# khuzema-h/marl-gym-pybullet-drones

Hardware: NVIDIA B200
Metric: drone_substeps_per_sec (higher is better)
Workload: dtype f32

## Files before the change

### marl_gym_pybullet_drones_b200/build.py

```python
from __future__ import annotations

import os
import shutil
import subprocess
import sys

_HERE = os.path.dirname(os.path.abspath(__file__))
CSRC = os.path.join(_HERE, "csrc")
SOURCES = [os.path.join(CSRC, "bd_kernels.cu"), os.path.join(CSRC, "bd_tile_launch.cu"), os.path.join(CSRC, "bd_api.cu"), os.path.join(CSRC, "bd_actor.cu"),
           os.path.join(CSRC, "bd_norm.cu"), os.path.join(CSRC, "bd_ppo.cu"), os.path.join(CSRC, "bd_peer.cu")]
HEADERS = [os.path.join(CSRC, "bd_params.h"), os.path.join(CSRC, "bd_device.cuh"), os.path.join(CSRC, "bd_step_tile.cuh"),
           os.path.join(CSRC, "bd_umma.cuh"),
           os.path.join(os.path.dirname(_HERE), "include", "batch_drones.h")]
OUT = os.path.join(_HERE, "libbatchdrones.so")

NVCC_FLAGS = [
    "-gencode", "arch=compute_100a,code=sm_100a",
    "-O3", "-lineinfo", "-std=c++17",
    "-Xcompiler", "-fPIC", "-shared",
]


def find_nvcc() -> str:
    cand = shutil.which("nvcc") or "/usr/local/cuda/bin/nvcc"
    if not os.path.exists(cand):
        raise RuntimeError("nvcc not found; cannot build the CUDA extension")
    return cand


def up_to_date() -> bool:
    if not os.path.exists(OUT):
        return False
    t = os.path.getmtime(OUT)
    return all(os.path.getmtime(p) <= t for p in SOURCES + HEADERS)


def build(force: bool = False, verbose: bool = False) -> str:
    if not force and up_to_date():
        return OUT
    from concurrent.futures import ThreadPoolExecutor
    nvcc = find_nvcc()
    objdir = os.path.join(CSRC, "_obj")
    os.makedirs(objdir, exist_ok=True)
    compile_flags = [f for f in NVCC_FLAGS if f != "-shared"]

    def compile_one(src):
        obj = os.path.join(objdir, os.path.basename(src)[:-3] + ".o")
        cmd = [nvcc] + compile_flags + (["-Xptxas", "-v"] if verbose else []) + ["-c", "-o", obj, src]
        res = subprocess.run(cmd, capture_output=True, text=True)
        if res.returncode != 0:
            raise RuntimeError("nvcc failed on " + src + ":\n" + res.stdout + res.stderr)
        if verbose:
            print(res.stderr)
        return obj

    with ThreadPoolExecutor(max_workers=len(SOURCES)) as pool:
        objs = list(pool.map(compile_one, SOURCES))
    res = subprocess.run([nvcc] + NVCC_FLAGS + ["-o", OUT] + objs, capture_output=True, text=True)
    if res.returncode != 0:
        raise RuntimeError("nvcc link failed:\n" + res.stdout + res.stderr)
    return OUT


if __name__ == "__main__":
    print(build(force="--force" in sys.argv, verbose="-v" in sys.argv))
```

### marl_gym_pybullet_drones_b200/csrc/bd_step_tile.cuh

```cuda
#pragma once
#include "bd_device.cuh"

namespace bd {

template <int A>
struct TileIn {
  float4 s0, s1, s2, s3;
  float4 act;
  int stepc;
  float ep_ret;
};

template <int A, bool HINT = false>
__device__ __forceinline__ void load_state(const Params<float>& P, long long g, int env, bool active, TileIn<A>& in,
                                           const L2Hints& h = L2Hints{}) {
  if (active) {
    if constexpr (HINT) {
      in.s0 = ld_hint(P.s0 + g, h.state); in.s1 = ld_hint(P.s1 + g, h.state);
      in.s2 = ld_hint(P.s2 + g, h.state); in.s3 = ld_hint(P.s3 + g, h.state);
      in.stepc = ld_hint(P.stepc + env, h.state);
      in.ep_ret = P.ep_ret != nullptr ? ld_hint(P.ep_ret + env, h.state) : 0.f;
    } else {
      in.s0 = P.s0[g]; in.s1 = P.s1[g]; in.s2 = P.s2[g]; in.s3 = P.s3[g];
      in.stepc = P.stepc[env];
      in.ep_ret = P.ep_ret != nullptr ? P.ep_ret[env] : 0.f;
    }
  } else {
    in.s0 = in.s1 = in.s2 = in.s3 = make_float4(0.f, 0.f, 0.f, 0.f);
    in.s1.z = 1.0f;
    in.stepc = 0;
    in.ep_ret = 0.f;
  }
}
template <int A, bool HINT = false>
__device__ __forceinline__ void load_action(const Params<float>& P, long long g, bool active, TileIn<A>& in,
                                            const L2Hints& h = L2Hints{}) {
  if (active) {
    if constexpr (HINT) {
      if constexpr (A == 4) in.act = ld_hint(reinterpret_cast<const float4*>(P.actions) + g, h.once);
      else in.act = make_float4(ld_hint(reinterpret_cast<const float*>(P.actions) + g, h.once), 0.f, 0.f, 0.f);
    } else {
      if constexpr (A == 4) in.act = reinterpret_cast<const float4*>(P.actions)[g];
      else in.act = make_float4(reinterpret_cast<const float*>(P.actions)[g], 0.f, 0.f, 0.f);
    }
  } else {
    in.act = make_float4(0.f, 0.f, 0.f, 0.f);
  }
}

__device__ __forceinline__ float swarm_reward_shfl(const Params<float>& P, const Drone<float>& d, float roll, float pitch,
                                                   int lane, int M, int drone, int& flags) {
  const unsigned full = 0xffffffffu;
  const int base = lane & ~(M - 1);
  const bool tilt = fabsf(roll) > .4f || fabsf(pitch) > .4f;
  flags = 0;
  float contrib = 0.f;
  if (P.task == TASK_MEETUP) {
    const int src = base | (M - 1 - drone);
    const float ox = __shfl_sync(full, d.px, src), oy = __shfl_sync(full, d.py, src), oz = __shfl_sync(full, d.pz, src);
    if (drone < M / 2) {
      const float dx = d.px - ox, dy = d.py - oy, dz = d.pz - oz;
      const float dist = sqrtf(dx * dx + dy * dy + dz * dz);
      contrib = (-1.f * (dist * dist)) * 2.f;
      if (dist > 0.1f) flags |= 4;
    }
    if (fabsf(d.px) > 5.0f || fabsf(d.py) > 5.0f || d.pz > 3.0f || d.pz < 0.1f || tilt) flags |= 2;
  } else if (P.task == TASK_LEADERFOLLOWER) {
    const float z0 = __shfl_sync(full, d.pz, base);
    if (drone == 0) {
      const float ex = 0.f - d.px, ey = 0.f - d.py, ez = 0.5f - d.pz;
      const float n = sqrtf(ex * ex + ey * ey + ez * ez);
      contrib = -1.f * (n * n);
    } else {
      const float dz = z0 - d.pz;
      const float n = sqrtf(dz * dz);
      contrib = -(1.f / (float)M) * (n * n);
    }
    if (fabsf(d.px) > 2.0f || fabsf(d.py) > 2.0f || d.pz > 2.0f || tilt) flags |= 2;
  } else {
    const float eps = 1e-3f;
    const float ni = sqrtf(d.vx * d.vx + d.vy * d.vy + d.vz * d.vz);
    float ali = 0.f, sp = 0.f;
#pragma unroll 1
    for (int o = 1; o < M; ++o) {
      const int src = base | ((lane + o) & (M - 1));
      const float ox = __shfl_sync(full, d.px, src), oy = __shfl_sync(full, d.py, src), oz = __shfl_sync(full, d.pz, src);
      const float ux = __shfl_sync(full, d.vx, src), uy = __shfl_sync(full, d.vy, src), uz = __shfl_sync(full, d.vz, src);
      const float nj = __shfl_sync(full, ni, src);
      const float dot = d.vx * ux + d.vy * uy + d.vz * uz;
      ali += dot / (ni + eps) / (nj + eps);
      const float dx = ox - d.px, dy = oy - d.py, dz = oz - d.pz;
      const float dist = sqrtf(dx * dx + dy * dy + dz * dz);
      sp = (o == 1 || dist < sp) ? dist : sp;
    }
    if (fabsf(d.px) > 10.0f || fabsf(d.py) > 10.0f || d.pz > 10.0f || tilt) flags |= 2;
    float cx = d.vx, cy = d.vy, cz = d.vz, ssp = sp;
#pragma unroll 1
    for (int o = M >> 1; o > 0; o >>= 1) {
      ali += __shfl_xor_sync(full, ali, o);
      cx += __shfl_xor_sync(full, cx, o); cy += __shfl_xor_sync(full, cy, o); cz += __shfl_xor_sync(full, cz, o);
      ssp += __shfl_xor_sync(full, ssp, o);
    }
    cx /= (float)M; cy /= (float)M; cz /= (float)M;
    const float speed = sqrtf(cx * cx + cy * cy + cz * cz);
    if (M == 1) return speed;
    const float avg = ssp / (float)M;
    float var = (sp - avg) * (sp - avg);
#pragma unroll 1
    for (int o = M >> 1; o > 0; o >>= 1) var += __shfl_xor_sync(full, var, o);
    var /= (float)M;
    float pen = 0.f;
    if (!(1.0f < avg && avg < 3.0f)) {
      const float a = fabsf(avg - 1.0f), b = fabsf(avg - 3.0f);
      pen = a < b ? a : b;
    }
    return ((ali / (float)(M * (M - 1)) + speed) - pen) - var;
  }
#pragma unroll 1
  for (int o = M >> 1; o > 0; o >>= 1) contrib += __shfl_xor_sync(full, contrib, o);
  return contrib;
}

template <int TASK, int A, bool VEC, int AERO>
__global__ void __launch_bounds__(kBlock, 6)
step_kernel_tile(const __grid_constant__ Params<float> P) {
  extern __shared__ __align__(128) unsigned char smem_raw[];
  const int tid = threadIdx.x, lane = tid & 31;
  const int M = P.M, B = P.B, D = P.D, EW = P.EW;
  const bool pow2 = (M & (M - 1)) == 0;
  constexpr bool vec = VEC;
  float* tile_s = reinterpret_cast<float*>(smem_raw);
  const int env_w = pow2 ? (lane >> (31 - __clz(M))) : lane / M;
  const int group_base = env_w * M;
  const int drone = lane - group_base;
  const int tile = blockIdx.x + P.block0;
  const int env_l = (tid >> 5) * EW + env_w;
  const int env = tile * (4 * EW) + env_l;
  const bool active = env_w < EW && env < P.N;
  const long long g0 = (long long)tile * (4 * EW) * M;
  const long long g = (long long)env * M + drone;
  float* myrow = tile_s + (size_t)(env_w < EW ? env_l * M + drone : 0) * D;
  const bool jit = (TASK == TASK_MULTIHOVER) && (P.reset_mode != RESET_FIXED);
  const long long gh = active ? g : P.n_total;
  const L2Hints l2 = l2_hints(P);

  pdl_launch_dependents();
  int total, head;
  const bool pipe = P.pipe_wait && P.host_total >= 0;
  if (pipe) {
    total = P.host_total;
    head = P.host_head;
    if (pipe_gate(P, tile, total, tid)) pdl_wait();
    issue_history<float, A, VEC, true>(P, gh, head, myrow, 0, B - 2, l2);
  } else if (P.host_total >= 0 && P.early_prefetch) {
    total = P.host_total;
    head = P.host_head;
    issue_history<float, A, VEC, true>(P, gh, head, myrow, 0, B - 2, l2);
    pdl_wait();
  } else {
    pdl_wait();
    total = P.host_total >= 0 ? P.host_total : P.gsteps[0];
    head = total % B;
    issue_history<float, A, VEC, true>(P, gh, head, myrow, 0, B - 2, l2);
  }
  TileIn<A> cur;
  load_state<A, true>(P, g, env, active, cur, l2);
  issue_history<float, A, VEC, true>(P, gh, head, myrow, B - 2, B - 1, l2);
  cp_async_commit();
  load_action<A, true>(P, g, active, cur, l2);
  const int stepc = cur.stepc;
  float last_sum = 0.f;
  if constexpr (AERO == 2) {
    if ((P.aero & AERO_DRAG) && active && stepc > 0) {
      const int prev = head == 0 ? B - 1 : head - 1;
      const float* lp = P.hist + ((size_t)prev * P.n_total + g) * A;
      if constexpr (A == 4) {
        const float4 pa = *reinterpret_cast<const float4*>(lp);
        last_sum = (__fadd_rn(1.0f, __fmul_rn(0.05f, pa.x)) + __fadd_rn(1.0f, __fmul_rn(0.05f, pa.y))) +
                   (__fadd_rn(1.0f, __fmul_rn(0.05f, pa.z)) + __fadd_rn(1.0f, __fmul_rn(0.05f, pa.w)));
      } else {
        last_sum = 4.0f * __fadd_rn(1.0f, __fmul_rn(0.05f, lp[0]));
      }
    }
  }

  Drone<float> d;
  d.px = cur.s0.x; d.py = cur.s0.y; d.pz = cur.s0.z; d.qx = cur.s0.w;
  d.qy = cur.s1.x; d.qz = cur.s1.y; d.qw = cur.s1.z; d.vx = cur.s1.w;
  d.vy = cur.s2.x; d.vz = cur.s2.y; d.wx = cur.s2.z; d.wy = cur.s2.w;
  d.wz = cur.s3.x; d.tx = cur.s3.y; d.ty = cur.s3.z; d.tz = cur.s3.w;
  float onep[4];
  if constexpr (A == 4) {
    onep[0] = __fadd_rn(1.0f, __fmul_rn(0.05f, cur.act.x));
    onep[1] = __fadd_rn(1.0f, __fmul_rn(0.05f, cur.act.y));
    onep[2] = __fadd_rn(1.0f, __fmul_rn(0.05f, cur.act.z));
    onep[3] = __fadd_rn(1.0f, __fmul_rn(0.05f, cur.act.w));
  } else {
    onep[0] = onep[1] = onep[2] = onep[3] = __fadd_rn(1.0f, __fmul_rn(0.05f, cur.act.x));
  }

  float avx = 0.f, avy = 0.f, avz = 0.f;
  fast_substeps<AERO>(P, d, onep, avx, avy, avz, group_base, drone, last_sum);
  float roll, pitch, yaw;
  quat_to_euler_fast(d.qx, d.qy, d.qz, d.qw, roll, pitch, yaw);

  cp_async_wait_all();
  float contrib = 0.f;
  int flags = 0;
  if (active) {
    if (vec) {
      float4* r4 = reinterpret_cast<float4*>(myrow);
      r4[0] = make_float4(d.px, d.py, d.pz, roll);
      r4[1] = make_float4(pitch, yaw, d.vx, d.vy);
      r4[2] = make_float4(d.vz, avx, avy, avz);
    } else {
      myrow[0] = d.px; myrow[1] = d.py; myrow[2] = d.pz; myrow[3] = roll; myrow[4] = pitch; myrow[5] = yaw;
      myrow[6] = d.vx; myrow[7] = d.vy; myrow[8] = d.vz; myrow[9] = avx; myrow[10] = avy; myrow[11] = avz;
    }
    if constexpr (TASK != TASK_SWARM)
      task_terms<float, TASK>(P, d, roll, pitch, stepc, drone, myrow + 12 + B * A, contrib, flags);
    if constexpr (A == 4) {
      if (vec) *reinterpret_cast<float4*>(myrow + 12 + (B - 1) * 4) = cur.act;
      else { float* o = myrow + 12 + (B - 1) * 4; o[0] = cur.act.x; o[1] = cur.act.y; o[2] = cur.act.z; o[3] = cur.act.w; }
      st_hint(reinterpret_cast<float4*>(P.hist + ((size_t)head * P.n_total + g) * 4), cur.act, l2_slot_pol(l2, 0));
    } else {
      myrow[12 + B - 1] = cur.act.x;
      st_hint(P.hist + (size_t)head * P.n_total + g, cur.act.x, l2_slot_pol(l2, 0));
    }
  }

  float swarm_reward_env = 0.f;
  if constexpr (TASK == TASK_SWARM) {
    int fl = 0;
    swarm_reward_env = swarm_reward_shfl(P, d, roll, pitch, lane, M, drone, fl);
    flags = active ? fl : 0;
  }
  if (pow2) {
#pragma unroll 1
    for (int o = M >> 1; o > 0; o >>= 1) {
      contrib += __shfl_xor_sync(0xffffffffu, contrib, o);
      flags |= __shfl_xor_sync(0xffffffffu, flags, o);
    }
  } else {
    const float c0 = contrib;
    const int f0 = flags;
#pragma unroll 1
    for (int o = 1; o < M; ++o) {
      int t = drone + o;
      t -= (t >= M) ? M : 0;
      contrib += __shfl_sync(0xffffffffu, c0, group_base + t);
      flags |= __shfl_sync(0xffffffffu, f0, group_base + t);
    }
  }
  const float reward = (TASK == TASK_SWARM) ? swarm_reward_env : ((TASK == TASK_HOVER) ? contrib : contrib / (float)M);
  const bool time_up = stepc >= P.trunc_counter;
  const bool terminated = (TASK == TASK_SWARM) ? (P.task == TASK_MEETUP && (flags & 4) == 0) : (flags & 1) != 0;
  const bool truncated = ((flags & 2) != 0) || time_up;
  const bool done_reset = active && (terminated || truncated) && P.auto_reset;
  if (active && drone == 0) {
    P.reward[env] = reward;
    P.terminated[env] = terminated ? 1 : 0;
    P.truncated[env] = truncated ? 1 : 0;
    st_hint(P.stepc + env, done_reset ? 0 : stepc + P.S, l2.state);
    if (P.ep_ret != nullptr) {
      float ep = cur.ep_ret + reward;
      if (terminated || truncated) {
        atomicAdd(P.ep_acc + 0, (double)ep);
        atomicAdd(P.ep_acc + 1, (double)(stepc / P.S + 1));
        atomicAdd(P.ep_acc + 2, 1.0);
        ep = 0.f;
      }
      st_hint(P.ep_ret + env, ep, l2.state);
    }
  }

  if (__any_sync(0xffffffffu, done_reset)) {
    float cx = 0.f, cy = 0.f, cz = 0.f;
    if (jit) {
      const long long ib = (long long)env * P.init_env_stride + drone * 3;
      bool retry = done_reset;
#pragma unroll 1
      for (int attempt = 0; attempt <= kMaxJitterTries; ++attempt) {
        const bool last = attempt == kMaxJitterTries;
        if (retry) {
          float j0 = 0.f, j1 = 0.f, j2 = 0.f;
          if (!last) {
            if (P.reset_mode == RESET_BUFFER && P.jitter != nullptr) {
              j0 = P.jitter[g * 3]; j1 = P.jitter[g * 3 + 1]; j2 = P.jitter[g * 3 + 2];
            } else {
              uint32_t c[4] = {(uint32_t)env, (uint32_t)total + P.philox_base, (uint32_t)(attempt * M + drone), 0u};
              uint32_t c2[4] = {c[0], c[1], c[2], 1u};
              philox4x32_10(c, (uint32_t)P.seed, (uint32_t)(P.seed >> 32));
              philox4x32_10(c2, (uint32_t)P.seed, (uint32_t)(P.seed >> 32));
              j0 = -0.25f + 0.5f * u01(c[0], c[1], 0.f);
              j1 = -0.25f + 0.5f * u01(c[2], c[3], 0.f);
              j2 = -0.25f + 0.5f * u01(c2[0], c2[1], 0.f);
            }
          }
          cx = P.init_xyz[ib] + j0;
          cy = P.init_xyz[ib + 1] + j1;
          cz = P.init_xyz[ib + 2] + j2;
          cz = cz < 0.1f ? 0.1f : (cz > 1.0f ? 1.0f : cz);
        }
        int bad = 0;
#pragma unroll 1
        for (int o = 1; o < M; ++o) {
          int t = drone + o;
          t -= (t >= M) ? M : 0;
          const int src = group_base + t;
          const float ox = __shfl_sync(0xffffffffu, cx, src), oy = __shfl_sync(0xffffffffu, cy, src),
                      oz = __shfl_sync(0xffffffffu, cz, src);
          const float dx = cx - ox, dy = cy - oy, dz = cz - oz;
          bad |= (sqrtf(dx * dx + dy * dy + dz * dz) < 0.5f) ? 1 : 0;
        }
        {
          const int b0 = bad;
#pragma unroll 1
          for (int o = 1; o < M; ++o) {
            int t = drone + o;
            t -= (t >= M) ? M : 0;
            bad |= __shfl_sync(0xffffffffu, b0, group_base + t);
          }
        }
        if (last || P.reset_mode == RESET_BUFFER) bad = 0;
        retry = retry && (bad != 0);
        if (!__any_sync(0xffffffffu, retry)) break;
      }
    }
    if (done_reset) {
      if (P.terminal_obs != nullptr) {
        float* to = P.terminal_obs + (size_t)g * D;
        for (int k = 0; k < D; ++k) to[k] = myrow[k];
      }
      const float cand[3] = {cx, cy, cz};
      float kin[12];
      reset_drone<float, TASK>(P, env, drone, jit ? cand : nullptr, d, kin);
#pragma unroll
      for (int k = 0; k < 12; ++k) myrow[k] = kin[k];
      if (TASK == TASK_SPIRAL) {
        float rp[3], rv[3], sphi, cphi;
        spiral_reference(P, 0, drone, rp, rv, sphi, cphi);
        spiral_extras(myrow + 12 + B * A, d, rp, rv, sphi, cphi);
      }
    }
  }

  const long long left = P.n_total - g0;
  const int tile_rows = 4 * EW * M;
  const int rows = (int)(left < (long long)tile_rows ? left : (long long)tile_rows);
  const uint32_t bytes = (uint32_t)rows * (uint32_t)D * 4u;
  float* gobs = P.obs + (size_t)g0 * D;
  const bool bulk = P.obs_aligned && (bytes & 15u) == 0;
  if (bulk) fence_proxy_async_smem();
  __syncthreads();
  if (bulk) {
    if (tid == 0) bulk_store_s2g(gobs, tile_s, bytes);
  } else {
    for (int i = tid; i < rows * D; i += kBlock) gobs[i] = tile_s[i];
  }
  if (active) {
    st_hint(P.s0 + g, make_float4(d.px, d.py, d.pz, d.qx), l2.state);
    st_hint(P.s1 + g, make_float4(d.qy, d.qz, d.qw, d.vx), l2.state);
    st_hint(P.s2 + g, make_float4(d.vy, d.vz, d.wx, d.wy), l2.state);
    st_hint(P.s3 + g, make_float4(d.wz, d.tx, d.ty, d.tz), l2.state);
  }
  if (P.pipeline) {
    __syncthreads();
    if (tid == 0) {
      if (bulk) bulk_wait_all0();
      if (P.host_total >= 0) {
        if (tile == 0) P.gsteps[0] = (total + 1 >= P.total_wrap) ? 0 : total + 1;
      } else {
        const unsigned ticket = atomicAdd(reinterpret_cast<unsigned*>(P.gsteps + 1), 1u);
        if (ticket == gridDim.x - 1) {
          P.gsteps[1] = 0;
          if (P.advance) P.gsteps[0] = (total + 1 >= P.total_wrap) ? 0 : total + 1;
        }
      }
      st_release_gpu(P.tile_epoch + tile, total + 1);
      atomicAdd(P.finished, 1ull);
    }
    return;
  }
  if (tid == 0) {
    const unsigned ticket = atomicAdd(reinterpret_cast<unsigned*>(P.gsteps + 1), 1u);
    if (ticket == gridDim.x - 1) {
      P.gsteps[1] = 0;
      if (P.advance) P.gsteps[0] = (total + 1 >= P.total_wrap) ? 0 : total + 1;
    }
    if (bulk) bulk_wait_read0();
  }
}


struct ManySpan {
  int K;
  long long act_step;
  long long obs_step;
  long long out_step;
};
__device__ __forceinline__ void bulk_wait_read1() { asm volatile("cp.async.bulk.wait_group.read 1;\n" ::: "memory"); }

template <int TASK, int A, bool VEC, int AERO>
__global__ void __launch_bounds__(kBlock, 3)
step_kernel_tile_many(const __grid_constant__ Params<float> P, const ManySpan Q) {
  extern __shared__ __align__(128) unsigned char smem_raw[];
  const int tid = threadIdx.x, lane = tid & 31;
  const int M = P.M, B = P.B, D = P.D, EW = P.EW;
  const bool pow2 = (M & (M - 1)) == 0;
  constexpr bool vec = VEC;
  const int env_w = pow2 ? (lane >> (31 - __clz(M))) : lane / M;
  const int group_base = env_w * M;
  const int drone = lane - group_base;
  const int tile = blockIdx.x;
  const int env_l = (tid >> 5) * EW + env_w;
  const int env = tile * (4 * EW) + env_l;
  const bool active = env_w < EW && env < P.N;
  const long long g0 = (long long)tile * (4 * EW) * M;
  const long long g = (long long)env * M + drone;
  const int tile_rows = 4 * EW * M;
  const size_t tile_floats = (size_t)tile_rows * D;
  float* const tiles = reinterpret_cast<float*>(smem_raw);
  const size_t rowoff = (size_t)(env_w < EW ? env_l * M + drone : 0) * D;
  const bool jit = (TASK == TASK_MULTIHOVER) && (P.reset_mode != RESET_FIXED);
  const long long gh = active ? g : P.n_total;
  const long long left = P.n_total - g0;
  const int rows = (int)(left < (long long)tile_rows ? left : (long long)tile_rows);
  const uint32_t bytes = (uint32_t)rows * (uint32_t)D * 4u;

  pdl_wait();
  int total = P.host_total >= 0 ? P.host_total : P.gsteps[0];
  int head = total % B;
  TileIn<A> cur;
  load_state<A>(P, g, env, active, cur);
  issue_history<float, A, VEC>(P, gh, head, tiles + rowoff, 0, B - 1);
  cp_async_commit();
  load_action<A>(P, g, active, cur);
  int stepc = cur.stepc;
  float ep = cur.ep_ret;
  float last_sum = 0.f;
  if constexpr (AERO == 2) {
    if ((P.aero & AERO_DRAG) && active && stepc > 0) {
      const int prev = head == 0 ? B - 1 : head - 1;
      const float* lp = P.hist + ((size_t)prev * P.n_total + g) * A;
      if constexpr (A == 4) {
        const float4 pa = *reinterpret_cast<const float4*>(lp);
        last_sum = (__fadd_rn(1.0f, __fmul_rn(0.05f, pa.x)) + __fadd_rn(1.0f, __fmul_rn(0.05f, pa.y))) +
                   (__fadd_rn(1.0f, __fmul_rn(0.05f, pa.z)) + __fadd_rn(1.0f, __fmul_rn(0.05f, pa.w)));
      } else {
        last_sum = 4.0f * __fadd_rn(1.0f, __fmul_rn(0.05f, lp[0]));
      }
    }
  }
  Drone<float> d;
  d.px = cur.s0.x; d.py = cur.s0.y; d.pz = cur.s0.z; d.qx = cur.s0.w;
  d.qy = cur.s1.x; d.qz = cur.s1.y; d.qw = cur.s1.z; d.vx = cur.s1.w;
  d.vy = cur.s2.x; d.vz = cur.s2.y; d.wx = cur.s2.z; d.wy = cur.s2.w;
  d.wz = cur.s3.x; d.tx = cur.s3.y; d.ty = cur.s3.z; d.tz = cur.s3.w;
  float4 act = cur.act;

#pragma unroll 1
  for (int k = 0; k < Q.K; ++k) {
    float* const tile_s = tiles + (size_t)(k & 1) * tile_floats;
    float* const myrow = tile_s + rowoff;
    float4 act_next = make_float4(0.f, 0.f, 0.f, 0.f);
    if (k + 1 < Q.K && active) {
      if constexpr (A == 4) act_next = reinterpret_cast<const float4*>(reinterpret_cast<const float*>(P.actions) + (size_t)(k + 1) * Q.act_step)[g];
      else act_next.x = (reinterpret_cast<const float*>(P.actions) + (size_t)(k + 1) * Q.act_step)[g];
    }
    if (k > 0) {
      if (k > 1) {
        if (tid == 0) bulk_wait_read1();
        __syncthreads();
      }
      const float* prow = tiles + (size_t)((k - 1) & 1) * tile_floats + rowoff;
      if (active) {
        if constexpr (A == 4) {
          if (vec) {
#pragma unroll 4
            for (int j = 0; j < B - 1; ++j)
              *reinterpret_cast<float4*>(myrow + 12 + j * 4) = *reinterpret_cast<const float4*>(prow + 12 + (j + 1) * 4);
          } else {
            for (int j = 0; j < (B - 1) * 4; ++j) myrow[12 + j] = prow[12 + 4 + j];
          }
        } else {
          for (int j = 0; j < B - 1; ++j) myrow[12 + j] = prow[12 + 1 + j];
        }
      }
    }
    float onep[4];
    if constexpr (A == 4) {
      onep[0] = __fadd_rn(1.0f, __fmul_rn(0.05f, act.x));
      onep[1] = __fadd_rn(1.0f, __fmul_rn(0.05f, act.y));
      onep[2] = __fadd_rn(1.0f, __fmul_rn(0.05f, act.z));
      onep[3] = __fadd_rn(1.0f, __fmul_rn(0.05f, act.w));
    } else {
      onep[0] = onep[1] = onep[2] = onep[3] = __fadd_rn(1.0f, __fmul_rn(0.05f, act.x));
    }
    float avx = 0.f, avy = 0.f, avz = 0.f;
    fast_substeps<AERO>(P, d, onep, avx, avy, avz, group_base, drone, last_sum);
    float roll, pitch, yaw;
    quat_to_euler_fast(d.qx, d.qy, d.qz, d.qw, roll, pitch, yaw);
    if (k == 0) cp_async_wait_all();
    float contrib = 0.f;
    int flags = 0;
    if (active) {
      if (vec) {
        float4* r4 = reinterpret_cast<float4*>(myrow);
        r4[0] = make_float4(d.px, d.py, d.pz, roll);
        r4[1] = make_float4(pitch, yaw, d.vx, d.vy);
        r4[2] = make_float4(d.vz, avx, avy, avz);
      } else {
        myrow[0] = d.px; myrow[1] = d.py; myrow[2] = d.pz; myrow[3] = roll; myrow[4] = pitch; myrow[5] = yaw;
        myrow[6] = d.vx; myrow[7] = d.vy; myrow[8] = d.vz; myrow[9] = avx; myrow[10] = avy; myrow[11] = avz;
      }
      if constexpr (TASK != TASK_SWARM)
        task_terms<float, TASK>(P, d, roll, pitch, stepc, drone, myrow + 12 + B * A, contrib, flags);
      if constexpr (A == 4) {
        if (vec) *reinterpret_cast<float4*>(myrow + 12 + (B - 1) * 4) = act;
        else { float* o = myrow + 12 + (B - 1) * 4; o[0] = act.x; o[1] = act.y; o[2] = act.z; o[3] = act.w; }
        *reinterpret_cast<float4*>(P.hist + ((size_t)head * P.n_total + g) * 4) = act;
      } else {
        myrow[12 + B - 1] = act.x;
        P.hist[(size_t)head * P.n_total + g] = act.x;
      }
    }
    float swarm_reward_env = 0.f;
    if constexpr (TASK == TASK_SWARM) {
      int fl = 0;
      swarm_reward_env = swarm_reward_shfl(P, d, roll, pitch, lane, M, drone, fl);
      flags = active ? fl : 0;
    }
    if (pow2) {
#pragma unroll 1
      for (int o = M >> 1; o > 0; o >>= 1) {
        contrib += __shfl_xor_sync(0xffffffffu, contrib, o);
        flags |= __shfl_xor_sync(0xffffffffu, flags, o);
      }
    } else {
      const float c0 = contrib;
      const int f0 = flags;
#pragma unroll 1
      for (int o = 1; o < M; ++o) {
        int t = drone + o;
        t -= (t >= M) ? M : 0;
        contrib += __shfl_sync(0xffffffffu, c0, group_base + t);
        flags |= __shfl_sync(0xffffffffu, f0, group_base + t);
      }
    }
    const float reward = (TASK == TASK_SWARM) ? swarm_reward_env : ((TASK == TASK_HOVER) ? contrib : contrib / (float)M);
    const bool time_up = stepc >= P.trunc_counter;
    const bool terminated = (TASK == TASK_SWARM) ? (P.task == TASK_MEETUP && (flags & 4) == 0) : (flags & 1) != 0;
    const bool truncated = ((flags & 2) != 0) || time_up;
    const bool done_reset = active && (terminated || truncated) && P.auto_reset;
    if (active && drone == 0) {
      const size_t o = (size_t)k * Q.out_step + env;
      P.reward[o] = reward;
      P.terminated[o] = terminated ? 1 : 0;
      P.truncated[o] = truncated ? 1 : 0;
      if (P.ep_ret != nullptr) {
        ep += reward;
        if (terminated || truncated) {
          atomicAdd(P.ep_acc + 0, (double)ep);
          atomicAdd(P.ep_acc + 1, (double)(stepc / P.S + 1));
          atomicAdd(P.ep_acc + 2, 1.0);
          ep = 0.f;
        }
      }
    }
    if constexpr (AERO == 2) last_sum = done_reset ? 0.f : (onep[0] + onep[1]) + (onep[2] + onep[3]);
    stepc = done_reset ? 0 : stepc + P.S;

    if (__any_sync(0xffffffffu, done_reset)) {
      float cx = 0.f, cy = 0.f, cz = 0.f;
      if (jit) {
        const long long ib = (long long)env * P.init_env_stride + drone * 3;
        bool retry = done_reset;
#pragma unroll 1
        for (int attempt = 0; attempt <= kMaxJitterTries; ++attempt) {
          const bool last = attempt == kMaxJitterTries;
          if (retry) {
            float j0 = 0.f, j1 = 0.f, j2 = 0.f;
            if (!last) {
              if (P.reset_mode == RESET_BUFFER && P.jitter != nullptr) {
                j0 = P.jitter[g * 3]; j1 = P.jitter[g * 3 + 1]; j2 = P.jitter[g * 3 + 2];
              } else {
                uint32_t c[4] = {(uint32_t)env, (uint32_t)total + P.philox_base, (uint32_t)(attempt * M + drone), 0u};
                uint32_t c2[4] = {c[0], c[1], c[2], 1u};
                philox4x32_10(c, (uint32_t)P.seed, (uint32_t)(P.seed >> 32));
                philox4x32_10(c2, (uint32_t)P.seed, (uint32_t)(P.seed >> 32));
                j0 = -0.25f + 0.5f * u01(c[0], c[1], 0.f);
                j1 = -0.25f + 0.5f * u01(c[2], c[3], 0.f);
                j2 = -0.25f + 0.5f * u01(c2[0], c2[1], 0.f);
              }
            }
            cx = P.init_xyz[ib] + j0;
            cy = P.init_xyz[ib + 1] + j1;
            cz = P.init_xyz[ib + 2] + j2;
            cz = cz < 0.1f ? 0.1f : (cz > 1.0f ? 1.0f : cz);
          }
          int bad = 0;
#pragma unroll 1
          for (int o = 1; o < M; ++o) {
            int t = drone + o;
            t -= (t >= M) ? M : 0;
            const int src = group_base + t;
            const float ox = __shfl_sync(0xffffffffu, cx, src), oy = __shfl_sync(0xffffffffu, cy, src),
                        oz = __shfl_sync(0xffffffffu, cz, src);
            const float dx = cx - ox, dy = cy - oy, dz = cz - oz;
            bad |= (sqrtf(dx * dx + dy * dy + dz * dz) < 0.5f) ? 1 : 0;
          }
          {
            const int b0 = bad;
#pragma unroll 1
            for (int o = 1; o < M; ++o) {
              int t = drone + o;
              t -= (t >= M) ? M : 0;
              bad |= __shfl_sync(0xffffffffu, b0, group_base + t);
            }
          }
          if (last || P.reset_mode == RESET_BUFFER) bad = 0;
          retry = retry && (bad != 0);
          if (!__any_sync(0xffffffffu, retry)) break;
        }
      }
      if (done_reset) {
        const float cand[3] = {cx, cy, cz};
        float kin[12];
        reset_drone<float, TASK>(P, env, drone, jit ? cand : nullptr, d, kin);
#pragma unroll
        for (int q = 0; q < 12; ++q) myrow[q] = kin[q];
        if (TASK == TASK_SPIRAL) {
          float rp[3], rv[3], sphi, cphi;
          spiral_reference(P, 0, drone, rp, rv, sphi, cphi);
          spiral_extras(myrow + 12 + B * A, d, rp, rv, sphi, cphi);
        }
      }
    }
    fence_proxy_async_smem();
    __syncthreads();
    if (tid == 0) bulk_store_s2g(P.obs + (size_t)k * Q.obs_step + (size_t)g0 * D, tile_s, bytes);
    act = act_next;
    total = (total + 1 >= P.total_wrap) ? 0 : total + 1;
    head = head + 1 == B ? 0 : head + 1;
  }

  if (active) {
    P.s0[g] = make_float4(d.px, d.py, d.pz, d.qx);
    P.s1[g] = make_float4(d.qy, d.qz, d.qw, d.vx);
    P.s2[g] = make_float4(d.vy, d.vz, d.wx, d.wy);
    P.s3[g] = make_float4(d.wz, d.tx, d.ty, d.tz);
    if (drone == 0) {
      P.stepc[env] = stepc;
      if (P.ep_ret != nullptr) P.ep_ret[env] = ep;
    }
  }
  __syncthreads();
  if (tid == 0) {
    bulk_wait_all0();
    if (P.host_total >= 0) {
      if (tile == 0) P.gsteps[0] = total;
    } else {
      const unsigned ticket = atomicAdd(reinterpret_cast<unsigned*>(P.gsteps + 1), 1u);
      if (ticket == gridDim.x - 1) { P.gsteps[1] = 0; P.gsteps[0] = total; }
    }
    if (P.pipeline) {
      st_release_gpu(P.tile_epoch + tile, total);
      atomicAdd(P.finished, (unsigned long long)Q.K);
    }
  }
}

}
```

### marl_gym_pybullet_drones_b200/csrc/bd_tile_launch.cu

```cuda
#include <cuda_runtime.h>
#include <math.h>
#include <stdint.h>

#include "bd_device.cuh"
#include "bd_params.h"
#include "bd_step_tile.cuh"

namespace bd {

template <int TASK, int A>
static cudaError_t launch_step_tile_t(const Params<float>& P, const LaunchSpec& ls, cudaStream_t st) {
  const int envs_per_tile = 4 * P.EW;
  const size_t smem = (size_t)envs_per_tile * P.M * P.D * 4;
  const bool vecrow = (A == 4) && (P.D % 4 == 0);
  const int aero = P.aero == 0 ? 0 : (P.aero == AERO_DW ? 1 : 2);
  void (*kern)(Params<float>);
  if (vecrow) kern = aero == 0 ? step_kernel_tile<TASK, A, (A == 4), 0> : (aero == 1 ? step_kernel_tile<TASK, A, (A == 4), 1> : step_kernel_tile<TASK, A, (A == 4), 2>);
  else kern = aero == 0 ? step_kernel_tile<TASK, A, false, 0> : (aero == 1 ? step_kernel_tile<TASK, A, false, 1> : step_kernel_tile<TASK, A, false, 2>);
  static size_t configured[6][64] = {{0}};
  size_t* const cfgd = configured[(vecrow ? 1 : 0) + 2 * aero];
  const int dv = ls.device & 63;
  if (smem > cfgd[dv]) {
    cudaError_t e = cudaFuncSetAttribute(kern, cudaFuncAttributeMaxDynamicSharedMemorySize, (int)smem);
    if (e != cudaSuccess) return e;
    cfgd[dv] = smem;
  }
  const int grid = P.grid_blocks > 0 ? P.grid_blocks : (P.N + envs_per_tile - 1) / envs_per_tile;
  static int per_sm[6][64] = {{0}};
  static size_t per_sm_smem[6][64] = {{0}};
  int& occ = per_sm[(vecrow ? 1 : 0) + 2 * aero][dv];
  if (occ == 0 || per_sm_smem[(vecrow ? 1 : 0) + 2 * aero][dv] != smem) {
    if (cudaOccupancyMaxActiveBlocksPerMultiprocessor(&occ, kern, kBlock, smem) != cudaSuccess || occ < 1) occ = 1;
    per_sm_smem[(vecrow ? 1 : 0) + 2 * aero][dv] = smem;
  }
  Params<float> Q = P;
  Q.early_prefetch = (P.early_prefetch && ls.pdl && grid >= occ * ls.sm_count) ? 1 : 0;
  Q.pipe_wait = (P.pipeline && ls.pdl && grid >= occ * ls.sm_count) ? 1 : 0;
  cudaLaunchConfig_t cfg = {};
  cfg.gridDim = dim3(grid);
  cfg.blockDim = dim3(kBlock);
  cfg.dynamicSmemBytes = smem;
  cfg.stream = st;
  cudaLaunchAttribute attr[1];
  attr[0].id = cudaLaunchAttributeProgrammaticStreamSerialization;
  attr[0].val.programmaticStreamSerializationAllowed = 1;
  cfg.attrs = attr;
  cfg.numAttrs = ls.pdl ? 1 : 0;
  return cudaLaunchKernelEx(&cfg, kern, Q);
}

template <int TASK, int A>
static cudaError_t launch_step_tile_many_t(const Params<float>& P, const ManySpan& span, const LaunchSpec& ls, cudaStream_t st) {
  const int envs_per_tile = 4 * P.EW;
  const size_t smem = 2 * (size_t)envs_per_tile * P.M * P.D * 4;
  const bool vecrow = (A == 4) && (P.D % 4 == 0);
  const int aero = P.aero == 0 ? 0 : (P.aero == AERO_DW ? 1 : 2);
  void (*kern)(Params<float>, ManySpan);
  if (vecrow) kern = aero == 0 ? step_kernel_tile_many<TASK, A, (A == 4), 0> : (aero == 1 ? step_kernel_tile_many<TASK, A, (A == 4), 1> : step_kernel_tile_many<TASK, A, (A == 4), 2>);
  else kern = aero == 0 ? step_kernel_tile_many<TASK, A, false, 0> : (aero == 1 ? step_kernel_tile_many<TASK, A, false, 1> : step_kernel_tile_many<TASK, A, false, 2>);
  static size_t configured[6][64] = {{0}};
  size_t* const cfgd = configured[(vecrow ? 1 : 0) + 2 * aero];
  const int dv = ls.device & 63;
  if (smem > cfgd[dv]) {
    cudaError_t e = cudaFuncSetAttribute(kern, cudaFuncAttributeMaxDynamicSharedMemorySize, (int)smem);
    if (e != cudaSuccess) return e;
    cfgd[dv] = smem;
  }
  const int grid = (P.N + envs_per_tile - 1) / envs_per_tile;
  kern<<<grid, kBlock, smem, st>>>(P, span);
  return cudaGetLastError();
}

template <int TASK>
static cudaError_t tile_many_a(int act_a, const Params<float>& P, const ManySpan& span, const LaunchSpec& ls, cudaStream_t st) {
  return act_a == 4 ? launch_step_tile_many_t<TASK, 4>(P, span, ls, st) : launch_step_tile_many_t<TASK, 1>(P, span, ls, st);
}

cudaError_t launch_step_tile_many(int task, int act_a, const Params<float>& P, int k, long long act_step, long long obs_step,
                                  long long out_step, const LaunchSpec& ls, cudaStream_t st) {
  ManySpan span;
  span.K = k; span.act_step = act_step; span.obs_step = obs_step; span.out_step = out_step;
  switch (task) {
    case TASK_HOVER: return tile_many_a<TASK_HOVER>(act_a, P, span, ls, st);
    case TASK_MULTIHOVER: return tile_many_a<TASK_MULTIHOVER>(act_a, P, span, ls, st);
    case TASK_SPIRAL: return tile_many_a<TASK_SPIRAL>(act_a, P, span, ls, st);
    default: return tile_many_a<TASK_SWARM>(act_a, P, span, ls, st);
  }
}

template <int TASK>
static cudaError_t tile_a(int act_a, const Params<float>& P, const LaunchSpec& ls, cudaStream_t st) {
  return act_a == 4 ? launch_step_tile_t<TASK, 4>(P, ls, st) : launch_step_tile_t<TASK, 1>(P, ls, st);
}

cudaError_t launch_step_tile(int task, int act_a, const Params<float>& P, const LaunchSpec& ls, cudaStream_t st) {
  switch (task) {
    case TASK_HOVER: return tile_a<TASK_HOVER>(act_a, P, ls, st);
    case TASK_MULTIHOVER: return tile_a<TASK_MULTIHOVER>(act_a, P, ls, st);
    case TASK_SPIRAL: return tile_a<TASK_SPIRAL>(act_a, P, ls, st);
    default: return tile_a<TASK_SWARM>(act_a, P, ls, st);
  }
}

}
```

Baseline: 65.06 billion.

## Defer history prefetch after state loads and use per-warp bulk observation stores

Reorders the history cp.async prefetch so that, outside the early-prefetch path, state and action loads are issued first and all history rows are fetched in one batch. In pipeline mode each warp now issues its own bulk shared-to-global observation store after a warp sync instead of a block-wide barrier, and each warp's lane 0 waits on its own bulk group. Optional compile-time trace stamps (clock64/globaltimer) and a build option for defines are added for profiling; they are off by default. The reordering may delay when history loads start, and per-warp bulk stores increase the number of TMA ops.

```diff
diff --git a/marl_gym_pybullet_drones_b200/build.py b/marl_gym_pybullet_drones_b200/build.py
--- a/marl_gym_pybullet_drones_b200/build.py
+++ b/marl_gym_pybullet_drones_b200/build.py
@@ -35,14 +35,14 @@
     return all(os.path.getmtime(p) <= t for p in SOURCES + HEADERS)
 
 
-def build(force: bool = False, verbose: bool = False) -> str:
-    if not force and up_to_date():
+def build(force: bool = False, verbose: bool = False, out: str = OUT, defines: tuple = ()) -> str:
+    if out == OUT and not force and up_to_date():
         return OUT
     from concurrent.futures import ThreadPoolExecutor
     nvcc = find_nvcc()
-    objdir = os.path.join(CSRC, "_obj")
+    objdir = os.path.join(CSRC, "_obj") if out == OUT else os.path.join(os.path.dirname(out), "_obj")
     os.makedirs(objdir, exist_ok=True)
-    compile_flags = [f for f in NVCC_FLAGS if f != "-shared"]
+    compile_flags = [f for f in NVCC_FLAGS if f != "-shared"] + [f"-D{d}" for d in defines]
 
     def compile_one(src):
         obj = os.path.join(objdir, os.path.basename(src)[:-3] + ".o")
@@ -56,10 +56,10 @@
 
     with ThreadPoolExecutor(max_workers=len(SOURCES)) as pool:
         objs = list(pool.map(compile_one, SOURCES))
-    res = subprocess.run([nvcc] + NVCC_FLAGS + ["-o", OUT] + objs, capture_output=True, text=True)
+    res = subprocess.run([nvcc] + NVCC_FLAGS + ["-o", out] + objs, capture_output=True, text=True)
     if res.returncode != 0:
         raise RuntimeError("nvcc link failed:\n" + res.stdout + res.stderr)
-    return OUT
+    return out
 
 
 if __name__ == "__main__":
diff --git a/marl_gym_pybullet_drones_b200/csrc/bd_step_tile.cuh b/marl_gym_pybullet_drones_b200/csrc/bd_step_tile.cuh
--- a/marl_gym_pybullet_drones_b200/csrc/bd_step_tile.cuh
+++ b/marl_gym_pybullet_drones_b200/csrc/bd_step_tile.cuh
@@ -2,6 +2,24 @@
 #include "bd_device.cuh"
 
 namespace bd {
+
+#ifdef BD_STEP_TRACE
+constexpr int kTraceLaunches = 4;
+__device__ long long* g_step_trace;
+__device__ __forceinline__ long long trace_globaltimer() {
+  long long t;
+  asm volatile("mov.u64 %0, %%globaltimer;" : "=l"(t));
+  return t;
+}
+#define BD_STAMP(k, v)                                     \
+  do {                                                     \
+    float dep_ = (v);                                      \
+    asm volatile("add.f32 %0, %0, 0f00000000;" : "+f"(dep_)); \
+    trace_t[k] = clock64() + (dep_ == 1.2345e-30f ? 1 : 0); \
+  } while (0)
+#else
+#define BD_STAMP(k, v) do {} while (0)
+#endif
 
 template <int A>
 struct TileIn {
@@ -143,16 +161,20 @@
   const bool jit = (TASK == TASK_MULTIHOVER) && (P.reset_mode != RESET_FIXED);
   const long long gh = active ? g : P.n_total;
   const L2Hints l2 = l2_hints(P);
+#ifdef BD_STEP_TRACE
+  long long trace_t[8] = {clock64(), 0, 0, 0, 0, 0, 0, 0};
+  const long long trace_g0 = trace_globaltimer();
+#endif
 
   pdl_launch_dependents();
   int total, head;
   const bool pipe = P.pipe_wait && P.host_total >= 0;
+  const bool early = !pipe && P.host_total >= 0 && P.early_prefetch;
   if (pipe) {
     total = P.host_total;
     head = P.host_head;
     if (pipe_gate(P, tile, total, tid)) pdl_wait();
-    issue_history<float, A, VEC, true>(P, gh, head, myrow, 0, B - 2, l2);
-  } else if (P.host_total >= 0 && P.early_prefetch) {
+  } else if (early) {
     total = P.host_total;
     head = P.host_head;
     issue_history<float, A, VEC, true>(P, gh, head, myrow, 0, B - 2, l2);
@@ -161,13 +183,19 @@
     pdl_wait();
     total = P.host_total >= 0 ? P.host_total : P.gsteps[0];
     head = total % B;
-    issue_history<float, A, VEC, true>(P, gh, head, myrow, 0, B - 2, l2);
-  }
+  }
+  BD_STAMP(1, (float)total);
   TileIn<A> cur;
   load_state<A, true>(P, g, env, active, cur, l2);
-  issue_history<float, A, VEC, true>(P, gh, head, myrow, B - 2, B - 1, l2);
-  cp_async_commit();
-  load_action<A, true>(P, g, active, cur, l2);
+  if (early) {
+    issue_history<float, A, VEC, true>(P, gh, head, myrow, B - 2, B - 1, l2);
+    cp_async_commit();
+    load_action<A, true>(P, g, active, cur, l2);
+  } else {
+    load_action<A, true>(P, g, active, cur, l2);
+    issue_history<float, A, VEC, true>(P, gh, head, myrow, 0, B - 1, l2);
+    cp_async_commit();
+  }
   const int stepc = cur.stepc;
   float last_sum = 0.f;
   if constexpr (AERO == 2) {
@@ -198,13 +226,16 @@
   } else {
     onep[0] = onep[1] = onep[2] = onep[3] = __fadd_rn(1.0f, __fmul_rn(0.05f, cur.act.x));
   }
+  BD_STAMP(2, ((cur.s0.x + cur.s1.x) + (cur.s2.x + cur.s3.x)) + (onep[0] + cur.ep_ret + (float)stepc));
 
   float avx = 0.f, avy = 0.f, avz = 0.f;
   fast_substeps<AERO>(P, d, onep, avx, avy, avz, group_base, drone, last_sum);
   float roll, pitch, yaw;
   quat_to_euler_fast(d.qx, d.qy, d.qz, d.qw, roll, pitch, yaw);
+  BD_STAMP(3, roll + pitch + yaw);
 
   cp_async_wait_all();
+  BD_STAMP(4, myrow[12]);
   float contrib = 0.f;
   int flags = 0;
   if (active) {
@@ -351,13 +382,43 @@
   const uint32_t bytes = (uint32_t)rows * (uint32_t)D * 4u;
   float* gobs = P.obs + (size_t)g0 * D;
   const bool bulk = P.obs_aligned && (bytes & 15u) == 0;
+#ifdef BD_STEP_TRACE
+  if (lane == 0 && g_step_trace != nullptr)
+    g_step_trace[((size_t)(total & (kTraceLaunches - 1)) * P.step_tiles + tile) * 16 + 12 + (tid >> 5)] = clock64();
+#endif
+  const int wrows_all = EW * M;
+  const bool warp_bulk = P.pipeline && bulk && ((wrows_all * D) & 3) == 0;
   if (bulk) fence_proxy_async_smem();
-  __syncthreads();
-  if (bulk) {
-    if (tid == 0) bulk_store_s2g(gobs, tile_s, bytes);
+  if (warp_bulk) {
+    const int r0 = (tid >> 5) * wrows_all;
+    const int wrows = min(max(rows - r0, 0), wrows_all);
+    __syncwarp();
+    if (lane == 0 && wrows > 0) bulk_store_s2g(gobs + (size_t)r0 * D, tile_s + (size_t)r0 * D, (uint32_t)wrows * D * 4u);
   } else {
-    for (int i = tid; i < rows * D; i += kBlock) gobs[i] = tile_s[i];
-  }
+    __syncthreads();
+    if (bulk) {
+      if (tid == 0) bulk_store_s2g(gobs, tile_s, bytes);
+    } else {
+      for (int i = tid; i < rows * D; i += kBlock) gobs[i] = tile_s[i];
+    }
+  }
+  BD_STAMP(5, 0.f);
+#ifdef BD_STEP_TRACE
+#define BD_TRACE_WRITE()                                                                                      \
+  do {                                                                                                        \
+    long long* tr_ = g_step_trace;                                                                            \
+    if (tr_ != nullptr) {                                                                                     \
+      tr_ += ((size_t)(total & (kTraceLaunches - 1)) * P.step_tiles + tile) * 16;                             \
+      trace_t[7] = clock64();                                                                                 \
+      for (int k_ = 0; k_ < 8; ++k_) tr_[k_] = trace_t[k_];                                                   \
+      tr_[8] = trace_g0; tr_[9] = trace_globaltimer();                                                        \
+      unsigned sm_; asm volatile("mov.u32 %0, %%smid;" : "=r"(sm_));                                          \
+      tr_[10] = sm_; tr_[11] = total;                                                                         \
+    }                                                                                                         \
+  } while (0)
+#else
+#define BD_TRACE_WRITE() do {} while (0)
+#endif
   if (active) {
     st_hint(P.s0 + g, make_float4(d.px, d.py, d.pz, d.qx), l2.state);
     st_hint(P.s1 + g, make_float4(d.qy, d.qz, d.qw, d.vx), l2.state);
@@ -365,9 +426,10 @@
     st_hint(P.s3 + g, make_float4(d.wz, d.tx, d.ty, d.tz), l2.state);
   }
   if (P.pipeline) {
+    if (bulk && lane == 0) bulk_wait_all0();
     __syncthreads();
     if (tid == 0) {
-      if (bulk) bulk_wait_all0();
+      BD_STAMP(6, 0.f);
       if (P.host_total >= 0) {
         if (tile == 0) P.gsteps[0] = (total + 1 >= P.total_wrap) ? 0 : total + 1;
       } else {
@@ -379,6 +441,7 @@
       }
       st_release_gpu(P.tile_epoch + tile, total + 1);
       atomicAdd(P.finished, 1ull);
+      BD_TRACE_WRITE();
     }
     return;
   }
@@ -389,8 +452,11 @@
       if (P.advance) P.gsteps[0] = (total + 1 >= P.total_wrap) ? 0 : total + 1;
     }
     if (bulk) bulk_wait_read0();
+    BD_STAMP(6, 0.f);
+    BD_TRACE_WRITE();
   }
 }
+#undef BD_TRACE_WRITE
 
 
 struct ManySpan {
diff --git a/marl_gym_pybullet_drones_b200/csrc/bd_tile_launch.cu b/marl_gym_pybullet_drones_b200/csrc/bd_tile_launch.cu
--- a/marl_gym_pybullet_drones_b200/csrc/bd_tile_launch.cu
+++ b/marl_gym_pybullet_drones_b200/csrc/bd_tile_launch.cu
@@ -103,3 +103,9 @@
 }
 
 }
+
+#ifdef BD_STEP_TRACE
+extern "C" int bd_step_set_trace(long long* trace_dev) {
+  return cudaMemcpyToSymbol(bd::g_step_trace, &trace_dev, sizeof(trace_dev)) == cudaSuccess ? 0 : 1;
+}
+#endif
```

Result: faster. 67.25 billion (median of 6 runs) (+3.4%).
